# TencentEMapReduce/alluxio

Hardware: AMD Instinct MI355X
Metric: StressWorkerBench cached seq-read GB/s (whole node) at 1/2/4/8 MI355X workers (higher is better)
Workload: dtype uint8; 1 GPU; model=StressWorkerBench cached seq-read, HBM MEM tier, global_batch=256, seq_len=4096, parallelism=workers1, threads_per_worker=256, block_size=67108864, buffer_size=4096, page_size=2097152, verified=True, headline_verified=True, full=False

## Files before the change

### alluxio_amd/csrc/bindings.cpp

```cpp
#include <pybind11/pybind11.h>
#include <pybind11/stl.h>
#include <pybind11/numpy.h>

#include <cmath>
#include <cstring>
#include <vector>

#include "block_store.h"
#include "trace.h"
#include "cpu_codecs.h"
#include "ipc.h"
#include "numa_host.h"
#include "ring_read.h"
#include "ragged_gather.h"
#include "delim_index.h"
#include "field_parse.h"
#include "kernels.h"
#include "seg_ring.h"
#include "frame_rpc.h"
#include "journal_log.h"
#include "meta_codec.h"
#include "fuse_server.h"
#include "http_blob.h"

// ... 820 lines not shown
      .def_property_readonly("passthrough_opens", &FuseServer::passthrough_opens)
      .def("stats", &FuseServer::stats)
      .def_property_readonly("native_opens", &FuseServer::native_opens)
      .def_property_readonly("native_reads", &FuseServer::native_reads)
      .def_property_readonly("fallback_opens", &FuseServer::fallback_opens);
  py::class_<JournalLog>(m, "JournalLog")
      .def(py::init<const std::string&, uint64_t, uint64_t, bool, double>(), py::arg("log_dir"),
           py::arg("next_seq"), py::arg("max_log_bytes"), py::arg("fsync") = true, py::arg("batch_ms") = 5.0)
      .def("append", [](JournalLog& j, py::bytes entry) {
             std::string e = entry;
             return j.append(e);
           })
      .def("request", &JournalLog::request)
      .def("wait_flushed", &JournalLog::wait_flushed, py::arg("counter"), py::arg("timeout_ms") = -1,
           py::call_guard<py::gil_scoped_release>())
      .def("reply_when_flushed", [](JournalLog& j, uint64_t counter, FrameRpcServer& srv, const py::tuple& t) {
             FrameReply r{t[0].cast<uint64_t>(), t[1].cast<int>(), t[2].cast<std::string>(),
                          std::string(t[3].cast<py::bytes>())};
             py::gil_scoped_release rel;
             j.reply_when_flushed(counter, &srv, std::move(r));
           })
      .def("close", &JournalLog::close, py::call_guard<py::gil_scoped_release>())
      .def_property_readonly("next_seq", &JournalLog::next_seq)
      .def_property_readonly("appended", &JournalLog::appended)
      .def_property_readonly("flushed", &JournalLog::flushed)
      .def_property_readonly("error", &JournalLog::error)
      .def_property_readonly("flushes", &JournalLog::flushes)
      .def_property_readonly("segments", &JournalLog::segments)
      .def("stats", &JournalLog::stats);

  py::class_<FrameRpcClient>(m, "FrameRpcClient")
      .def(py::init<const std::string&, int, const std::string&, int>(), py::arg("host"), py::arg("port"),
           py::arg("auth"), py::arg("timeout_ms") = 60000)
      .def("call", [](FrameRpcClient& c, const std::string& path, py::bytes payload, int timeout_ms) {
             std::string p = payload;
             std::tuple<int, std::string, std::string> r;
             {
               py::gil_scoped_release rel;
               r = c.call(path, p, timeout_ms);
             }
             return py::make_tuple(std::get<0>(r), py::str(std::get<1>(r)), py::bytes(std::get<2>(r)));
           }, py::arg("path"), py::arg("payload"), py::arg("timeout_ms") = 0)
      .def("close", &FrameRpcClient::close, G());
  bind_data_path(m);

  m.def("device_count", &hip_device_count);

  m.def("ipc_export", [](uint64_t ptr) {
          IpcExport e = ipc_export(ptr);
          return py::make_tuple(py::bytes(e.handle), e.offset, e.alloc_bytes);
        }, py::arg("ptr"));
  m.def("ipc_open", [](py::bytes handle, int device) {
          std::string h = handle;
          py::gil_scoped_release rel;
          return ipc_open(h, device);
        }, py::arg("handle"), py::arg("device"));
  m.def("ipc_open_bounded", [](py::bytes handle, int device, int timeout_ms) {
          std::string h = handle;
          py::gil_scoped_release rel;
          return ipc_open_bounded(h, device, timeout_ms);
        }, py::arg("handle"), py::arg("device"), py::arg("timeout_ms"));
  py::register_exception<IpcTimeout>(m, "IpcTimeout", PyExc_TimeoutError);
  m.def("ipc_close", [](uint64_t base) { py::gil_scoped_release rel; ipc_close(base); });
  m.def("gpu_numa_node", &gpu_numa_node, py::arg("device"));
  m.def("process_placement", &process_placement);
  m.def("device_arena_alloc", [](uint64_t bytes, int device) {
          py::gil_scoped_release rel;
          return device_arena_alloc(bytes, device);
        }, py::arg("bytes"), py::arg("device"));
  m.def("device_arena_free", [](uint64_t ptr, int device) {
          py::gil_scoped_release rel;
          device_arena_free(ptr, device);
        }, py::arg("ptr"), py::arg("device"));
  m.def("enable_peer_access", &enable_peer_access, py::arg("device"), py::arg("peer"));
  m.def("host_register", [](uint64_t ptr, uint64_t n) {
          if (hip_device_count() == 0) return false;
          HIP_CHECK(hipHostRegister(reinterpret_cast<void*>(ptr), n, hipHostRegisterMapped));
          return true;
        }, py::arg("ptr"), py::arg("nbytes"));
  m.def("host_unregister", [](uint64_t ptr) {
          if (hip_device_count() > 0) (void)hipHostUnregister(reinterpret_cast<void*>(ptr));
        }, py::arg("ptr"));
  m.def("can_access_peer", &can_access_peer, py::arg("device"), py::arg("peer"));
  m.def("crc32c", [](py::buffer data, uint32_t crc) {
          py::buffer_info bi = data.request();
          const size_t n = static_cast<size_t>(bi.size) * bi.itemsize;
          py::gil_scoped_release rel;
          return crc32c_sw(bi.ptr, n, crc);
        }, py::arg("data"), py::arg("crc") = 0);
  m.def("crc32c_ptr", [](uint64_t ptr, uint64_t n, uint32_t crc) {
          py::gil_scoped_release rel;
          return crc32c_sw(reinterpret_cast<const void*>(ptr), n, crc);
        }, py::arg("ptr"), py::arg("n"), py::arg("crc") = 0);
  m.def("crc32c_chunks", [](py::buffer data, uint32_t bpc) {
          py::buffer_info bi = data.request();
          const auto* p = static_cast<const uint8_t*>(bi.ptr);
          const size_t n = static_cast<size_t>(bi.size) * bi.itemsize;
          if (bpc == 0) throw StoreError(kErrInvalidArgument, "bytes_per_checksum must be > 0");
          const size_t nc = (n + bpc - 1) / bpc;
          std::string out(nc * 4, '\0');
          {
            py::gil_scoped_release rel;
            for (size_t i = 0; i < nc; ++i) {
              const size_t off = i * bpc;
              const uint32_t c = crc32c_sw(p + off, std::min<size_t>(bpc, n - off), 0);
              out[4 * i] = char(c >> 24); out[4 * i + 1] = char(c >> 16);
              out[4 * i + 2] = char(c >> 8); out[4 * i + 3] = char(c);
            }
          }
          return py::bytes(out);
        }, py::arg("data"), py::arg("bytes_per_checksum") = 512);
  m.def("crc32c_combine", &crc32c_combine);
  m.def("crc32c_device_pages", &crc32c_device_pages, G(), py::arg("base"), py::arg("pages"), py::arg("length"),
        py::arg("page_bytes"));
  m.def("crc32c_device", &crc32c_device, G(), py::arg("ptr"), py::arg("length"), py::arg("piece") = 0,
        py::arg("stream") = 0);
  m.def("lz4_compress", [](py::bytes data) {
          std::string s = data;
          std::string out(lz4_compress_bound(s.size()), '\0');
          int64_t n;
          {
            py::gil_scoped_release rel;
            n = lz4_compress_block((const uint8_t*)s.data(), s.size(), (uint8_t*)&out[0], out.size());
          }
          if (n < 0) throw StoreError(kErrInvalidArgument, "lz4 compression failed");
          out.resize((size_t)n);
          return py::bytes(out);
        });
  m.def("lz4_decompress", [](py::bytes data, size_t capacity) {
          std::string s = data;
          std::string out(capacity, '\0');
          int64_t n;
          {
            py::gil_scoped_release rel;
            n = lz4_decompress_block((const uint8_t*)s.data(), s.size(), (uint8_t*)&out[0], out.size());
          }
          if (n < 0) throw StoreError(kErrInvalidArgument, "malformed lz4 block (" + std::to_string(n) + ")");
          out.resize((size_t)n);
          return py::bytes(out);
        });
  m.def("lz4_compress_bound", &lz4_compress_bound);
  m.def("trace_push", [](const std::string& name) { roctxRangePushA(name.c_str()); }, py::arg("name"));
  m.def("trace_pop", [] { roctxRangePop(); });
  m.def("trace_mark", [](const std::string& name) { roctxMarkA(name.c_str()); }, py::arg("name"));
  m.def("lz4_device", &lz4_device, G(), py::arg("chunks"), py::arg("compress"), py::arg("stream") = 0);
  m.def("lz4_device_kernel_ms", &lz4_device_kernel_ms, G(), py::arg("chunks"), py::arg("compress"),
        py::arg("reps") = 5);
  m.def("batched_copy", &batched_copy, G(), py::arg("segments"), py::arg("stream") = 0, py::arg("sync") = true);
  m.def("fill_pattern", [](uint64_t ptr, uint64_t bytes, uint64_t seed, uint64_t word_offset, uint64_t stream) {
          py::gil_scoped_release rel;
          HIP_CHECK(launch_fill_pattern(reinterpret_cast<uint8_t*>(ptr), bytes, seed, word_offset,
                                        reinterpret_cast<hipStream_t>(stream)));
        }, py::arg("ptr"), py::arg("bytes"), py::arg("seed"), py::arg("word_offset") = 0, py::arg("stream") = 0);
  m.def("evict_select_device", &evict_select_device);
  m.def("page_alloc_device", &page_alloc_device);
  m.def("set_copy_variant", &set_copy_variant, py::arg("variant"), py::arg("grid_cap") = 0);
  m.def("copy_variant", [] {
    int v = 0;
    unsigned cap = 0;
    copy_variant(&v, &cap);
    return py::make_tuple(v, cap);
  });
  m.def("set_crc_variant", &set_crc_variant, py::arg("variant"));
  m.def("set_lz4_decode_variant", &set_lz4_decode_variant, py::arg("variant"));
  m.def("set_lz4_encode_variant", &set_lz4_encode_variant, py::arg("variant"));
  m.def("set_seq_read_variant", &set_seq_read_variant, py::arg("variant"), py::arg("grid_cap") = 0);
  m.def("seq_read_variant", [] {
    int v = 0;
    unsigned cap = 0;
    seq_read_variant(&v, &cap);
    return py::make_tuple(v, cap);
  });
  m.def("set_ragged_gather_variant", &set_ragged_gather_variant, py::arg("variant"), py::arg("chunk_shift") = 0);
  m.def("ragged_gather_chunk_shift", &ragged_gather_chunk_shift);
  m.def("set_delim_index_variant", &set_delim_index_variant, py::arg("variant"), py::arg("tile_shift") = 0);
  m.def("delim_index_tile_shift", &delim_index_tile_shift);
  m.def("delim_index_variant", &delim_index_variant);
  m.def("set_delim_quote_variant", &set_delim_quote_variant, py::arg("variant"));
  m.def("delim_quote_variant", &delim_quote_variant);
  m.def("set_field_parse_variant", &set_field_parse_variant, py::arg("variant"));
  m.def("field_parse_variant", &field_parse_variant);
  m.def("set_page_gather_chunk_variant", &set_page_gather_chunk_variant, py::arg("variant"));
  m.attr("COPY_CHUNK") = kCopyChunk;
}
```

### alluxio_amd/csrc/kernels.h

```cpp
#pragma once
#include <hip/hip_runtime.h>
#include <cstddef>
#include <cstdint>

#include "field_parse_host.h"

namespace amdx {

struct CopySeg {
  uint64_t src;
  uint64_t dst;
  uint64_t bytes;
  uint64_t chunk0;
};

constexpr uint64_t kCopyChunk = 256 * 1024;

hipError_t launch_batched_copy(const CopySeg* segs, int nseg, uint64_t total_chunks,
                               hipStream_t stream);
void set_copy_variant(int variant, unsigned grid_cap);
void copy_variant(int* variant, unsigned* grid_cap);

struct SeqReadArgs {
  const uint8_t* arena;
  const int64_t* ftab;
  const uint64_t* c_init;
  uint8_t* dst;
  uint64_t stream_stride;
  uint64_t file_len;
  uint64_t buf;
  uint64_t launch_base;
  uint32_t cycle;
  uint32_t streams;
  uint32_t depth;
  uint32_t page_shift;
  uint64_t footprint = 0;
};
constexpr uint32_t kSeqReadMaxStreams = 8192;
hipError_t launch_seq_read(const SeqReadArgs& a, hipStream_t stream);
void set_seq_read_variant(int variant, unsigned grid_cap);
void seq_read_variant(int* variant, unsigned* grid_cap);

struct RaggedRow {
  uint64_t src;
  uint64_t dst_off;
  uint64_t span;
  uint32_t len;
  uint32_t chunk0;
};
struct RaggedRec {
  uint64_t start;
  uint32_t len;
  uint32_t pad;
};
struct RaggedGatherArgs {
  const uint8_t* arena;
  const int64_t* vtab;
  const RaggedRec* recs;
  const int64_t* idx;
  uint8_t* dst;
  uint64_t* out_off;
  uint32_t* out_len;
  RaggedRow* rows;
  uint32_t* chunk_pre;
  uint64_t n_rec;
  uint64_t row_stride;
  uint32_t batch;
  uint32_t page_shift;
  uint32_t align;
  uint32_t max_len;
  uint32_t padded;
  uint32_t pad_value;
  uint32_t total_chunks;
  uint32_t chunk_shift;
};
constexpr uint32_t kRaggedGatherMaxBatch = 65536;
hipError_t launch_ragged_gather(const RaggedGatherArgs& a, hipStream_t stream);
void set_ragged_gather_variant(int variant, unsigned chunk_shift);
uint32_t ragged_gather_chunk_shift();

struct DelimIndexArgs {
  const uint8_t* arena;
  const int64_t* vtab;
  uint32_t* tile_count;
  uint64_t* tile_base;
  uint64_t* out;
  uint64_t out_cap;
  uint64_t vstart;
  uint64_t bytes;
  uint64_t add;
  uint32_t ntiles;
  uint32_t page_shift;
  uint32_t tile_shift;
  uint32_t delim;
  uint32_t quote;
  uint32_t in_quote;
  uint32_t* tile_count_odd;
  uint32_t* tile_parity;
};
uint64_t delim_index_tiles(uint64_t vstart, uint64_t bytes, uint32_t tile_shift);
hipError_t launch_delim_count(const DelimIndexArgs& a, hipStream_t stream);
hipError_t launch_delim_scan(const DelimIndexArgs& a, hipStream_t stream);
hipError_t launch_delim_emit(const DelimIndexArgs& a, uint64_t total, hipStream_t stream);
hipError_t launch_delim_count_quoted(const DelimIndexArgs& a, hipStream_t stream);
hipError_t launch_delim_scan_quoted(const DelimIndexArgs& a, hipStream_t stream);
hipError_t launch_delim_emit_quoted(const DelimIndexArgs& a, uint64_t total, hipStream_t stream);
void set_delim_quote_variant(int variant);
int delim_quote_variant();
void set_delim_index_variant(int variant, unsigned tile_shift);
uint32_t delim_index_tile_shift();
int delim_index_variant();

hipError_t launch_field_parse(const FieldParseArgs& a, hipStream_t stream);
void set_field_parse_variant(int variant);
int field_parse_variant();

hipError_t launch_crc32c_pieces(const uint8_t* base, uint64_t total_bytes, uint64_t piece_bytes,
                                uint32_t* out, uint32_t* scratch, uint64_t scratch_words,
                                hipStream_t stream);
hipError_t launch_crc32c_pages(const uint8_t* base, const int64_t* page_idx, uint64_t total_bytes,
                               uint64_t page_bytes, uint32_t* out, uint32_t* scratch, uint64_t scratch_words,
                               hipStream_t stream);
uint64_t crc32c_pages_scratch_words(uint64_t total_bytes, uint64_t page_bytes);
hipError_t launch_crc32c_gather(const uint64_t* ptrs, const uint32_t* lens, uint64_t n, uint32_t* out,
                                hipStream_t stream);
uint64_t crc32c_gather_max_piece();
void set_crc_variant(int v);
uint64_t crc32c_scratch_words(uint64_t total_bytes, uint64_t piece_bytes);

struct Lz4Chunk {
  uint64_t src;
  uint64_t dst;
  uint32_t src_bytes;
  uint32_t dst_capacity;
};
hipError_t launch_lz4_decompress(const Lz4Chunk* chunks, int n, int32_t* out_sizes,
                                 hipStream_t stream);
void set_lz4_decode_variant(int v);
void set_lz4_encode_variant(int v);
hipError_t launch_lz4_compress(const Lz4Chunk* chunks, int n, int32_t* out_sizes,
                               hipStream_t stream);

struct EvictState {
  float* crf;
  uint64_t* last;
  uint64_t* fbytes;
  int32_t* dir;
  uint32_t n;
  uint64_t now;
  float step;
  float log2_inv_att;
  int policy;
  uint64_t dir_mask;
  int unit;
  int invert;
};
constexpr uint32_t kSlotSetState = 1, kSlotReset = 2, kSlotTouch = 4;
struct SlotUpdate {
  uint32_t slot;
  uint32_t flags;
  int32_t dir;
  float crf;
  uint64_t fbytes;
  uint64_t t;
};
constexpr unsigned kEvSlabRows = 128;
struct EvictCtl {
  unsigned long long hist[256];
  unsigned long long total;
  unsigned long long acc;
  unsigned long long tie_acc;
  unsigned long long freed;
  uint32_t prefix, mask;
  uint32_t all, done;
  uint32_t count, pad;
};
hipError_t launch_slot_update(const EvictState& st, const SlotUpdate* upd, uint32_t n, hipStream_t stream);
hipError_t launch_evict_select_grid(const EvictState& st, uint32_t target_dir, const uint32_t* excl,
                                    uint64_t need, uint32_t* keys, EvictCtl* ctl, uint32_t* out_slots,
                                    hipStream_t stream);
hipError_t launch_page_alloc(uint64_t* bits, uint32_t nwords, uint32_t want, uint32_t* partial,
                             int64_t* pages_out, uint32_t* claimed, hipStream_t stream);
uint32_t page_alloc_partials(uint32_t nwords);

struct ClaimItem {
  uint64_t src;
  uint64_t len;
  uint32_t want;
  uint32_t page_base;
  uint32_t chunk_base;
  uint32_t pad;
};
hipError_t launch_mag_fill(uint64_t* bits, uint32_t nwords, const uint64_t* upd, uint32_t n, hipStream_t stream);
hipError_t launch_mag_drain(uint64_t* bits, uint32_t nwords, uint64_t* out, hipStream_t stream);
// ... 88 lines not shown
```

### alluxio_amd/csrc/kernels.hip

```cpp
#include "kernels.h"

#include <algorithm>
#include <cstring>
#include <mutex>

namespace amdx {

constexpr int kCopyThreads = 256;
typedef unsigned int u32x4 __attribute__((ext_vector_type(4)));

template <int P>
__device__ __forceinline__ u32x4 ld16(const u32x4* p) {
  if constexpr (P == 1) return __builtin_nontemporal_load(p);
  else return *p;
}
template <int P>
__device__ __forceinline__ void st16(u32x4* p, u32x4 v) {
  if constexpr (P == 1) __builtin_nontemporal_store(v, p);
  else *p = v;
}

__device__ __forceinline__ void copy_bytes(const uint8_t* __restrict__ s, uint8_t* __restrict__ d,
                                           uint64_t n, int tid) {
  for (uint64_t i = tid; i < n; i += kCopyThreads) d[i] = s[i];
}

template <int UNROLL, int LP, int SP>
__device__ __forceinline__ void copy_range(uint64_t src, uint64_t dst, uint64_t n, int tid) {
  if (((src | dst) & 15) == 0) {
    const u32x4* __restrict__ s = reinterpret_cast<const u32x4*>(src);
    u32x4* __restrict__ d = reinterpret_cast<u32x4*>(dst);
    const uint64_t n16 = n >> 4;
    uint64_t i = tid;
    constexpr uint64_t kStep = (uint64_t)kCopyThreads * UNROLL;
    for (; i + (UNROLL - 1) * kCopyThreads < n16; i += kStep) {
      u32x4 v[UNROLL];
#pragma unroll
      for (int u = 0; u < UNROLL; ++u) v[u] = ld16<LP>(s + i + (uint64_t)u * kCopyThreads);
#pragma unroll
      for (int u = 0; u < UNROLL; ++u) st16<SP>(d + i + (uint64_t)u * kCopyThreads, v[u]);
    }
    for (; i < n16; i += kCopyThreads) st16<SP>(d + i, ld16<LP>(s + i));
    const uint64_t done = n16 << 4;
    if (done < n) copy_bytes(reinterpret_cast<const uint8_t*>(src) + done,
                             reinterpret_cast<uint8_t*>(dst) + done, n - done, tid);
  } else if (((src | dst) & 3) == 0) {
    const uint32_t* __restrict__ s = reinterpret_cast<const uint32_t*>(src);
    uint32_t* __restrict__ d = reinterpret_cast<uint32_t*>(dst);
    const uint64_t n4 = n >> 2;
    for (uint64_t i = tid; i < n4; i += kCopyThreads) d[i] = s[i];
    const uint64_t done = n4 << 2;
    if (done < n) copy_bytes(reinterpret_cast<const uint8_t*>(src) + done,
                             reinterpret_cast<uint8_t*>(dst) + done, n - done, tid);
  } else {
    copy_bytes(reinterpret_cast<const uint8_t*>(src), reinterpret_cast<uint8_t*>(dst), n, tid);
  }
}

template <int UNROLL, int LP, int SP>
__global__ __launch_bounds__(kCopyThreads) void batched_copy_kernel(
    const CopySeg* __restrict__ segs, int nseg, uint64_t total_chunks) {
  const int tid = threadIdx.x;
  for (uint64_t c = blockIdx.x; c < total_chunks; c += gridDim.x) {
    int lo = 0, hi = nseg - 1;
    while (lo < hi) {
      const int mid = (lo + hi + 1) >> 1;
      if (segs[mid].chunk0 <= c) lo = mid; else hi = mid - 1;
    }
    lo = __builtin_amdgcn_readfirstlane(lo);
    const uint64_t src = segs[lo].src, dst = segs[lo].dst, bytes = segs[lo].bytes;
    const uint64_t off = (c - segs[lo].chunk0) * kCopyChunk;
    const uint64_t n = bytes - off < kCopyChunk ? bytes - off : kCopyChunk;
    copy_range<UNROLL, LP, SP>(src + off, dst + off, n, tid);
  }
}

static int g_copy_variant = 8;
static unsigned g_copy_grid_cap = 4096;

void set_copy_variant(int variant, unsigned grid_cap) {
  g_copy_variant = variant;
  if (grid_cap) g_copy_grid_cap = grid_cap;
}
void copy_variant(int* variant, unsigned* grid_cap) {
  *variant = g_copy_variant;
  *grid_cap = g_copy_grid_cap;
}

hipError_t launch_batched_copy(const CopySeg* segs, int nseg, uint64_t total_chunks,
                               hipStream_t stream) {
  if (nseg <= 0 || total_chunks == 0) return hipSuccess;
  const dim3 grid((unsigned)std::min<uint64_t>(total_chunks, g_copy_grid_cap));
  const dim3 block(kCopyThreads);
#define AMDX_COPY(U, L, S) hipLaunchKernelGGL((batched_copy_kernel<U, L, S>), grid, block, 0, stream, segs, nseg, total_chunks)
  switch (g_copy_variant) {
    case 1: AMDX_COPY(8, 0, 1); break;
    case 2: AMDX_COPY(8, 1, 0); break;
    case 3: AMDX_COPY(8, 1, 1); break;
    case 4: AMDX_COPY(4, 0, 0); break;
    case 5: AMDX_COPY(4, 0, 1); break;
    case 8: AMDX_COPY(16, 0, 0); break;
    case 9: AMDX_COPY(16, 0, 1); break;
    default: AMDX_COPY(8, 0, 0); break;
  }
#undef AMDX_COPY
  return hipGetLastError();
}

constexpr int kSeqThreads = 256;

template <bool POW2, int UNROLL, int SP, int LP>
__global__ __launch_bounds__(kSeqThreads) void seq_read_kernel(SeqReadArgs a, uint32_t vpr_shift,
                                                               uint32_t depth_shift) {
  extern __shared__ uint32_t c0[];
  for (uint32_t s = threadIdx.x; s < a.streams; s += kSeqThreads)
    c0[s] = (uint32_t)((a.c_init[s] + a.launch_base) % a.cycle);
  __syncthreads();
  const uint64_t vpr = a.buf >> 4;
  const uint64_t nvec = (uint64_t)a.streams * a.depth * vpr;
  const uint64_t pmask = (1ull << a.page_shift) - 1;
  const uint64_t gstride = (uint64_t)gridDim.x * kSeqThreads;
  for (uint64_t base = (uint64_t)blockIdx.x * kSeqThreads + threadIdx.x; base < nvec;
       base += gstride * UNROLL) {
    u32x4 v[UNROLL];
    uint8_t* d[UNROLL];
    uint32_t nb[UNROLL];
#pragma unroll
    for (int u = 0; u < UNROLL; ++u) {
      const uint64_t i = base + (uint64_t)u * gstride;
      nb[u] = 0;
      d[u] = nullptr;
      if (i >= nvec) continue;
      uint64_t r, vi;
      uint32_t s, k;
      if constexpr (POW2) {
        r = i >> vpr_shift;
        vi = i & (vpr - 1);
        s = (uint32_t)(r >> depth_shift);
        k = (uint32_t)(r & (a.depth - 1));
      } else {
        r = i / vpr;
        vi = i - r * vpr;
        s = (uint32_t)(r / a.depth);
        k = (uint32_t)(r - (uint64_t)s * a.depth);
      }
      uint32_t c = c0[s] + k;
      if (c >= a.cycle) c = (uint32_t)(((uint64_t)c0[s] + k) % a.cycle);
      if (c == a.cycle - 1) continue;
      const uint64_t off = (uint64_t)c * a.buf + vi * 16;
      const uint64_t rend = ((uint64_t)c + 1) * a.buf;
      const uint64_t end = rend < a.file_len ? rend : a.file_len;
      if (off >= end) continue;
      const uint64_t page = (uint64_t)a.ftab[off >> a.page_shift];
      const uint8_t* src = a.arena + (page << a.page_shift) + (off & pmask);
      d[u] = a.dst + (uint64_t)s * a.stream_stride + (uint64_t)k * a.buf + vi * 16;
      if (end - off >= 16) {
        nb[u] = 16;
        v[u] = ld16<LP>(reinterpret_cast<const u32x4*>(src));
      } else {
        nb[u] = (uint32_t)(end - off);
        for (uint32_t b = 0; b < nb[u]; ++b) {
          const uint64_t o = off + b;
          d[u][b] = a.arena[((uint64_t)a.ftab[o >> a.page_shift] << a.page_shift) + (o & pmask)];
        }
      }
    }
#pragma unroll
    for (int u = 0; u < UNROLL; ++u)
      if (nb[u] == 16) st16<SP>(reinterpret_cast<u32x4*>(d[u]), v[u]);
  }
}

static int g_seq_variant = -1;
static unsigned g_seq_grid_cap = 8192;

void set_seq_read_variant(int variant, unsigned grid_cap) {
  g_seq_variant = variant;
  if (grid_cap) g_seq_grid_cap = grid_cap;
}
void seq_read_variant(int* variant, unsigned* grid_cap) {
  *variant = g_seq_variant;
  *grid_cap = g_seq_grid_cap;
}

static inline bool is_pow2(uint64_t x) { return x && !(x & (x - 1)); }
static inline uint32_t log2u(uint64_t x) {
  uint32_t s = 0;
  while ((1ull << s) < x) ++s;
  return s;
}

hipError_t launch_seq_read(const SeqReadArgs& a, hipStream_t stream) {
  if (a.streams == 0 || a.depth == 0 || a.buf == 0 || a.file_len == 0) return hipSuccess;
  if (a.streams > kSeqReadMaxStreams || (a.buf & 15) || (a.stream_stride & 15) ||
      ((uint64_t)a.dst & 15) || ((uint64_t)a.arena & 15))
    return hipErrorInvalidValue;
  const uint64_t vpr = a.buf >> 4;
  const uint64_t nvec = (uint64_t)a.streams * a.depth * vpr;
  const uint64_t fp = a.footprint ? a.footprint : a.file_len;
  const int var = g_seq_variant >= 0 ? g_seq_variant : (fp >= (128ull << 20) ? 4 : 0);
  const int unroll = (var & 2) ? 16 : 8;
  uint64_t blocks = (nvec + (uint64_t)kSeqThreads * unroll - 1) / ((uint64_t)kSeqThreads * unroll);
  if (blocks > g_seq_grid_cap) blocks = g_seq_grid_cap;
  if (blocks < 1) blocks = 1;
  const bool p2 = is_pow2(vpr) && is_pow2(a.depth);
  const uint32_t vs = log2u(vpr), ds = log2u(a.depth);
  const size_t lds = a.streams * sizeof(uint32_t);
  const dim3 g((unsigned)blocks), b(kSeqThreads);
#define AMDX_SEQ(P2, U, SP, LP) \
  hipLaunchKernelGGL((seq_read_kernel<P2, U, SP, LP>), g, b, lds, stream, a, vs, ds)
  const int sp = var & 1, lp = (var >> 2) & 1;
  if (p2) {
    if (unroll == 16) {
      if (lp) { if (sp) AMDX_SEQ(true, 16, 1, 1); else AMDX_SEQ(true, 16, 0, 1); }
      else { if (sp) AMDX_SEQ(true, 16, 1, 0); else AMDX_SEQ(true, 16, 0, 0); }
    } else {
      if (lp) { if (sp) AMDX_SEQ(true, 8, 1, 1); else AMDX_SEQ(true, 8, 0, 1); }
      else { if (sp) AMDX_SEQ(true, 8, 1, 0); else AMDX_SEQ(true, 8, 0, 0); }
    }
  } else {
    if (lp) { if (sp) AMDX_SEQ(false, 8, 1, 1); else AMDX_SEQ(false, 8, 0, 1); }
    else { if (sp) AMDX_SEQ(false, 8, 1, 0); else AMDX_SEQ(false, 8, 0, 0); }
  }
#undef AMDX_SEQ
  return hipGetLastError();
}

constexpr uint32_t kCrcPoly = 0x82F63B78u;
constexpr uint64_t kCrcSeg = 64 * 1024;
constexpr int kCrcThreads = 256;
constexpr uint64_t kCrcLane = kCrcSeg / kCrcThreads;

__constant__ uint32_t c_crc_tab[8][256];
__constant__ uint32_t c_x2n[64];
__constant__ uint32_t c_crc16[16][256];
__constant__ uint32_t c_shift4k[4][256];
__constant__ uint32_t c_lane_shift[256];
constexpr int kCrc4Threads = 1024;
__constant__ uint32_t c_crc11[12][2048];
__constant__ uint32_t c_shift16k[4][256];
__constant__ uint32_t c_lane_shift1k[kCrc4Threads];
constexpr int kCrc5Threads = 1024;
constexpr uint64_t kCrc5Chunk = 64;
__constant__ uint32_t c_shift5[4][256];
__constant__ uint32_t c_lane_shift5[kCrc5Threads];

static void host_crc_tables(uint32_t tab[8][256], uint32_t x2n[64]) {
  for (uint32_t i = 0; i < 256; ++i) {
    uint32_t c = i;
    for (int k = 0; k < 8; ++k) c = (c & 1) ? (c >> 1) ^ kCrcPoly : c >> 1;
    tab[0][i] = c;
  }
  for (int t = 1; t < 8; ++t)
    for (uint32_t i = 0; i < 256; ++i) tab[t][i] = (tab[t - 1][i] >> 8) ^ tab[0][tab[t - 1][i] & 0xFF];
  auto mult = [](uint32_t a, uint32_t b) {
    uint32_t m = 1u << 31, p = 0;
    for (;;) {
      if (a & m) { p ^= b; if ((a & (m - 1)) == 0) break; }
      m >>= 1;
      b = (b & 1) ? (b >> 1) ^ kCrcPoly : b >> 1;
    }
    return p;
  };
  uint32_t p = 1u << 30;
  x2n[0] = p;
  for (int k = 1; k < 64; ++k) { p = mult(p, p); x2n[k] = p; }
}

static uint32_t host_gf2_mult(uint32_t a, uint32_t b) {
  uint32_t p = 0;
  for (uint32_t m = 1u << 31; m; m >>= 1) {
    if (a & m) p ^= b;
    b = (b & 1) ? (b >> 1) ^ kCrcPoly : b >> 1;
  }
  return p;
}

static void host_crc16_tables(const uint32_t tab8[8][256], const uint32_t x2n[64], uint32_t t16[16][256],
                              uint32_t sh[4][256]) {
  for (uint32_t i = 0; i < 256; ++i) t16[0][i] = tab8[0][i];
  for (int t = 1; t < 16; ++t)
    for (uint32_t i = 0; i < 256; ++i) t16[t][i] = (t16[t - 1][i] >> 8) ^ t16[0][t16[t - 1][i] & 0xFF];
  const uint32_t k = x2n[15];
  for (int b = 0; b < 4; ++b)
    for (uint32_t i = 0; i < 256; ++i) sh[b][i] = host_gf2_mult(k, i << (8 * b));
}

static std::once_flag g_crc_once;
static hipError_t g_crc_init_err = hipSuccess;

static hipError_t ensure_crc_tables() {
  std::call_once(g_crc_once, [] {
    static uint32_t tab[8][256];
    static uint32_t x2n[64];
    host_crc_tables(tab, x2n);
    static uint32_t t16[16][256];
    static uint32_t sh[4][256];
    host_crc16_tables(tab, x2n, t16, sh);
    g_crc_init_err = hipMemcpyToSymbol(HIP_SYMBOL(c_crc_tab), tab, sizeof(tab));
    if (g_crc_init_err == hipSuccess)
      g_crc_init_err = hipMemcpyToSymbol(HIP_SYMBOL(c_x2n), x2n, sizeof(x2n));
    if (g_crc_init_err == hipSuccess)
      g_crc_init_err = hipMemcpyToSymbol(HIP_SYMBOL(c_crc16), t16, sizeof(t16));
    if (g_crc_init_err == hipSuccess)
      g_crc_init_err = hipMemcpyToSymbol(HIP_SYMBOL(c_shift4k), sh, sizeof(sh));
    static uint32_t t11[12][2048];
    uint32_t e[128];
    for (int k = 0; k < 128; ++k) e[k] = t16[15 - k / 8][1u << (k % 8)];
    for (int c = 0; c < 12; ++c)
      for (uint32_t v = 0; v < 2048; ++v) {
        uint32_t x = 0;
        for (int b = 0; b < 11; ++b)
          if (((v >> b) & 1) && 11 * c + b < 128) x ^= e[11 * c + b];
        t11[c][v] = x;
      }
    static uint32_t sh16k[4][256];
    for (int b = 0; b < 4; ++b)
      for (uint32_t i = 0; i < 256; ++i) sh16k[b][i] = host_gf2_mult(x2n[17], i << (8 * b));
    static uint32_t lane1k[kCrc4Threads];
    lane1k[0] = 1u << 31;
    for (int k = 1; k < kCrc4Threads; ++k) lane1k[k] = host_gf2_mult(lane1k[k - 1], x2n[7]);
    if (g_crc_init_err == hipSuccess)
      g_crc_init_err = hipMemcpyToSymbol(HIP_SYMBOL(c_crc11), t11, sizeof(t11));
    if (g_crc_init_err == hipSuccess)
      g_crc_init_err = hipMemcpyToSymbol(HIP_SYMBOL(c_shift16k), sh16k, sizeof(sh16k));
    if (g_crc_init_err == hipSuccess)
      g_crc_init_err = hipMemcpyToSymbol(HIP_SYMBOL(c_lane_shift1k), lane1k, sizeof(lane1k));
    {
      const uint64_t nbits = 8ull * (kCrc5Threads - 1) * kCrc5Chunk;
      uint32_t k5 = 1u << 31;
      for (int b = 0; b < 64; ++b)
        if ((nbits >> b) & 1) k5 = host_gf2_mult(x2n[b], k5);
      static uint32_t sh5[4][256];
      for (int b = 0; b < 4; ++b)
        for (uint32_t i = 0; i < 256; ++i) sh5[b][i] = host_gf2_mult(k5, i << (8 * b));
      static uint32_t lane5[kCrc5Threads];
      lane5[0] = 1u << 31;
      for (int d = 1; d < kCrc5Threads; ++d) lane5[d] = host_gf2_mult(lane5[d - 1], x2n[9]);
      if (g_crc_init_err == hipSuccess)
        g_crc_init_err = hipMemcpyToSymbol(HIP_SYMBOL(c_shift5), sh5, sizeof(sh5));
      if (g_crc_init_err == hipSuccess)
        g_crc_init_err = hipMemcpyToSymbol(HIP_SYMBOL(c_lane_shift5), lane5, sizeof(lane5));
    }
    static uint32_t lane_shift[256];
    lane_shift[0] = 1u << 31;
    for (int k = 1; k < 256; ++k) lane_shift[k] = host_gf2_mult(lane_shift[k - 1], x2n[7]);
    if (g_crc_init_err == hipSuccess)
      g_crc_init_err = hipMemcpyToSymbol(HIP_SYMBOL(c_lane_shift), lane_shift, sizeof(lane_shift));
  });
  return g_crc_init_err;
}

__device__ __forceinline__ uint32_t gf2_mult(uint32_t a, uint32_t b) {
  uint32_t m = 1u << 31, p = 0;
  for (int i = 0; i < 32; ++i) {
    if (a & m) p ^= b;
    m >>= 1;
    b = (b & 1) ? (b >> 1) ^ kCrcPoly : b >> 1;
  }
  return p;
}

__device__ __forceinline__ uint32_t xpow8n(uint64_t nbytes) {
  uint64_t n = nbytes << 3;
  uint32_t p = 1u << 31;
  int k = 0;
  while (n) {
    if (n & 1) p = gf2_mult(c_x2n[k & 63], p);
    n >>= 1;
    ++k;
  }
  return p;
}

__global__ __launch_bounds__(kCrcThreads) void crc32c_segments_kernel(
    const uint8_t* __restrict__ base, uint64_t total_bytes, uint64_t piece_bytes,
    uint64_t segs_per_piece, uint64_t nsegs, uint32_t* __restrict__ seg_crc) {
// ... 2453 lines not shown
```

### alluxio_amd/csrc/ring_read.cpp

```cpp
#include "ring_read.h"

#include <algorithm>
#include <cstring>
#include <string>

#include "kernels.h"

namespace amdx {

RingReadSession::RingReadSession(BlockStore* store, int64_t session, const std::vector<int64_t>& block_ids,
                                 const std::vector<uint64_t>& block_lens, uint64_t dst_base,
                                 uint64_t stream_stride, uint64_t buf_bytes, uint32_t depth, uint32_t streams,
                                 int dst_kind, const std::vector<uint64_t>& start_offsets)
    : store_(store), session_(session), blocks_(block_ids), pins_(store), buf_(buf_bytes), stride_(stream_stride),
      dst_(dst_base), depth_(depth), streams_(streams), kind_(dst_kind) {
  if (block_ids.size() != block_lens.size() || block_ids.empty())
    throw StoreError(kErrInvalidArgument, "ring read: bad block list");
  for (uint64_t l : block_lens) file_len_ += l;
  check_shape();
  view_.append_file(store_, pins_, session_, blocks_, block_lens, "ring read");
  on_device_ = store_->has_device();
  finish_init(start_offsets);
}

RingReadSession::RingReadSession(uint64_t arena_base, const std::vector<int64_t>& file_pages, uint64_t page_size,
                                 uint64_t file_len, int device, uint64_t dst_base, uint64_t stream_stride,
                                 uint64_t buf_bytes, uint32_t depth, uint32_t streams, int dst_kind,
                                 const std::vector<uint64_t>& start_offsets)
    : store_(nullptr), session_(0), pins_(nullptr), file_len_(file_len), buf_(buf_bytes), stride_(stream_stride),
      dst_(dst_base), depth_(depth), streams_(streams), kind_(dst_kind), on_device_(device >= 0), device_(device) {
  check_shape();
  view_ = PagedView::raw(arena_base, file_pages, page_size, device, "ring read");
  if (view_.vtab.size() < (file_len_ + page_size - 1) / page_size)
    throw StoreError(kErrInvalidArgument, "ring read: page table shorter than the file");
  finish_init(start_offsets);
}

void RingReadSession::check_shape() {
  if (buf_ == 0 || depth_ == 0 || streams_ == 0 || streams_ > kSeqReadMaxStreams)
    throw StoreError(kErrInvalidArgument, "ring read: bad buffer/depth/stream count");
  if (stride_ < (uint64_t)depth_ * buf_) throw StoreError(kErrInvalidArgument, "ring read: stride too small");
  if (file_len_ == 0) throw StoreError(kErrInvalidArgument, "ring read: empty file");
  const uint64_t calls = (file_len_ + buf_ - 1) / buf_;
  if (calls + 1 >= (1ull << 32)) throw StoreError(kErrInvalidArgument, "ring read: too many calls per pass");
  cycle_ = (uint32_t)(calls + 1);
}

void RingReadSession::set_device() const {
  if (store_) store_->use_device();
  else if (device_ >= 0) AMDX_HIP(hipSetDevice(device_));
}

void RingReadSession::finish_init(const std::vector<uint64_t>& start_offsets) {
  c_init_.assign(streams_, 0);
  for (uint32_t s = 0; s < streams_ && s < start_offsets.size(); ++s) {
    if (start_offsets[s] % buf_) throw StoreError(kErrInvalidArgument, "ring read: start offsets must be buffer aligned");
    c_init_[s] = std::min<uint64_t>(start_offsets[s] / buf_, cycle_ - 1);
  }
  std::vector<uint64_t> starts(c_init_);
  std::sort(starts.begin(), starts.end());
  const uint64_t distinct = (uint64_t)(std::unique(starts.begin(), starts.end()) - starts.begin());
  footprint_ = std::min<uint64_t>(file_len_, distinct * depth_ * buf_);
  if (on_device_) {
    if (buf_ & 15 || stride_ & 15 || dst_ & 15)
      throw StoreError(kErrInvalidArgument, "ring read: buffer size, stride and ring base must be 16-byte aligned");
    set_device();
    d_ftab_.alloc(view_.vtab.size() * sizeof(int64_t));
    d_cinit_.alloc(c_init_.size() * sizeof(uint64_t));
    AMDX_HIP(hipMemcpy(d_ftab_.p, view_.vtab.data(), view_.vtab.size() * sizeof(int64_t), hipMemcpyHostToDevice));
    AMDX_HIP(hipMemcpy(d_cinit_.p, c_init_.data(), c_init_.size() * sizeof(uint64_t), hipMemcpyHostToDevice));
  }
}

RingReadSession::~RingReadSession() {
  try {
    close();
  } catch (...) {
  }
}

void RingReadSession::close() {
  if (closed_) return;
  closed_ = true;
  d_ftab_.reset();
  d_cinit_.reset();
  pins_.release();
}

uint64_t RingReadSession::bytes_before(uint64_t g) const {
  const uint64_t passes = g / cycle_, rem = g % cycle_;
  return passes * file_len_ + std::min<uint64_t>(rem * buf_, file_len_);
}

uint64_t RingReadSession::step(uint64_t stream, uint64_t* eofs) {
  if (closed_) throw StoreError(kErrInvalidState, "ring read session closed");
  const uint64_t base = calls_per_stream_;
  if (on_device_) {
    set_device();
    SeqReadArgs a;
    a.arena = view_.base();
    a.ftab = d_ftab_.as<int64_t>();
    a.c_init = d_cinit_.as<uint64_t>();
    a.dst = reinterpret_cast<uint8_t*>(dst_);
    a.stream_stride = stride_;
    a.file_len = file_len_;
    a.buf = buf_;
    a.launch_base = base;
    a.cycle = cycle_;
    a.streams = streams_;
    a.depth = depth_;
    a.page_shift = view_.page_shift;
    a.footprint = footprint_;
    hipStream_t st = reinterpret_cast<hipStream_t>(stream);
    AMDX_HIP(launch_seq_read(a, st));
    if (kind_ == (int)MemKind::kHost) AMDX_HIP(hipStreamSynchronize(st));
  } else {
    for (uint32_t s = 0; s < streams_; ++s)
      for (uint32_t k = 0; k < depth_; ++k) {
        auto [off, len] = std::pair<uint64_t, uint64_t>(0, 0);
        const uint64_t c = (c_init_[s] + base + k) % cycle_;
        if (c == cycle_ - 1) continue;
        off = c * buf_;
        len = std::min(buf_, file_len_ - off);
        uint8_t* d = reinterpret_cast<uint8_t*>(dst_ + s * stride_ + (uint64_t)k * buf_);
        for_each_page_run(view_.base(), view_.vtab.data(), view_.page_shift, off, len,
                          [d](const uint8_t* p, uint64_t n, uint64_t done) { std::memcpy(d + done, p, n); });
      }
  }
  uint64_t bytes = 0, eof = 0;
  for (uint32_t s = 0; s < streams_; ++s) {
    const uint64_t g0 = c_init_[s] + base, g1 = g0 + depth_;
    bytes += bytes_before(g1) - bytes_before(g0);
    eof += g1 / cycle_ - g0 / cycle_;
  }
  calls_per_stream_ += depth_;
  total_ += bytes;
  reopens_ += eof;
  if (store_) store_->access_blocks(blocks_);
  if (eofs) *eofs = eof;
  return bytes;
}

uint64_t RingReadSession::position(uint32_t s) const {
  const uint64_t c = (c_init_.at(s) + calls_per_stream_) % cycle_;
  return std::min<uint64_t>(c * buf_, file_len_);
}

std::pair<uint64_t, uint64_t> RingReadSession::last_call(uint32_t s, uint32_t k) const {
  if (calls_per_stream_ < depth_) return {0, 0};
  const uint64_t c = (c_init_.at(s) + calls_per_stream_ - depth_ + k) % cycle_;
  if (c == cycle_ - 1) return {file_len_, 0};
  const uint64_t off = c * buf_;
  return {off, std::min(buf_, file_len_ - off)};
}

}
```

### alluxio_amd/csrc/ring_read.h

```cpp
#pragma once
#include <cstdint>
#include <vector>

#include "paged_view.h"

namespace amdx {

class RingReadSession {
 public:
  RingReadSession(BlockStore* store, int64_t session, const std::vector<int64_t>& block_ids,
                  const std::vector<uint64_t>& block_lens, uint64_t dst_base, uint64_t stream_stride,
                  uint64_t buf_bytes, uint32_t depth, uint32_t streams, int dst_kind,
                  const std::vector<uint64_t>& start_offsets);
  RingReadSession(uint64_t arena_base, const std::vector<int64_t>& file_pages, uint64_t page_size,
                  uint64_t file_len, int device, uint64_t dst_base, uint64_t stream_stride, uint64_t buf_bytes,
                  uint32_t depth, uint32_t streams, int dst_kind, const std::vector<uint64_t>& start_offsets);
  ~RingReadSession();
  uint64_t step(uint64_t stream, uint64_t* eofs);
  void close();
  uint64_t total_bytes() const { return total_; }
  uint64_t reopens() const { return reopens_; }
  uint64_t calls() const { return calls_per_stream_; }
  uint64_t position(uint32_t s) const;
  std::pair<uint64_t, uint64_t> last_call(uint32_t s, uint32_t k) const;
  uint64_t file_len() const { return file_len_; }

 private:
  uint64_t bytes_before(uint64_t g) const;
  void check_shape();
  void finish_init(const std::vector<uint64_t>& start_offsets);
  void set_device() const;
  BlockStore* store_;
  int64_t session_;
  std::vector<int64_t> blocks_;
  BlockPins pins_;
  uint64_t file_len_ = 0, buf_, stride_, dst_;
  uint32_t depth_, streams_, cycle_;
  int kind_;
  bool on_device_ = false;
  int device_ = -1;
  PagedView view_;
  std::vector<uint64_t> c_init_;
  uint64_t footprint_ = 0;
  DevBuf d_ftab_, d_cinit_;
  uint64_t calls_per_stream_ = 0, total_ = 0, reopens_ = 0;
  bool closed_ = false;
};

}
```

Before: 5878 GB/s.

## Add wave-per-chunk fast seq-read kernel with persistent grid and modular call base

Adds a new seq-read kernel in which each wavefront copies U contiguous 1 KiB chunks. When the run stays inside one page and one call, a single page-table lookup serves all U loads; otherwise it falls back to a per-chunk path. The grid is capped at the occupancy-derived resident workgroup count, and the host keeps a modular base so the kernel avoids 64-bit modulo per element. It also computes the byte accounting in a closed form for lockstep streams and adds a store-fill probe kernel, at the cost of many extra template instantiations and more complex index arithmetic.

Result: faster. 6510 GB/s, median of 6 (+10.8%).

```diff
diff --git a/alluxio_amd/csrc/bindings.cpp b/alluxio_amd/csrc/bindings.cpp
--- a/alluxio_amd/csrc/bindings.cpp
+++ b/alluxio_amd/csrc/bindings.cpp
@@ -996,6 +996,15 @@
           HIP_CHECK(launch_fill_pattern(reinterpret_cast<uint8_t*>(ptr), bytes, seed, word_offset,
                                         reinterpret_cast<hipStream_t>(stream)));
         }, py::arg("ptr"), py::arg("bytes"), py::arg("seed"), py::arg("word_offset") = 0, py::arg("stream") = 0);
+  m.def("store_fill", [](uint64_t ptr, uint64_t bytes, uint32_t word, bool nontemporal, unsigned grid,
+                         uint64_t stream) {
+          py::gil_scoped_release rel;
+          unsigned used = 0;
+          HIP_CHECK(launch_store_fill(reinterpret_cast<uint8_t*>(ptr), bytes, word, nontemporal, grid, &used,
+                                      reinterpret_cast<hipStream_t>(stream)));
+          return used;
+        }, py::arg("ptr"), py::arg("bytes"), py::arg("word") = 0, py::arg("nontemporal") = false,
+        py::arg("grid") = 0, py::arg("stream") = 0);
   m.def("evict_select_device", &evict_select_device);
   m.def("page_alloc_device", &page_alloc_device);
   m.def("set_copy_variant", &set_copy_variant, py::arg("variant"), py::arg("grid_cap") = 0);
@@ -1015,6 +1024,10 @@
     seq_read_variant(&v, &cap);
     return py::make_tuple(v, cap);
   });
+  m.def("seq_read_last_launch", [] {
+    const SeqReadLaunch l = seq_read_last_launch();
+    return py::make_tuple(l.fast ? "fast" : "general", l.unroll, l.grid);
+  });
   m.def("set_ragged_gather_variant", &set_ragged_gather_variant, py::arg("variant"), py::arg("chunk_shift") = 0);
   m.def("ragged_gather_chunk_shift", &ragged_gather_chunk_shift);
   m.def("set_delim_index_variant", &set_delim_index_variant, py::arg("variant"), py::arg("tile_shift") = 0);
diff --git a/alluxio_amd/csrc/kernels.h b/alluxio_amd/csrc/kernels.h
--- a/alluxio_amd/csrc/kernels.h
+++ b/alluxio_amd/csrc/kernels.h
@@ -35,11 +35,20 @@
   uint32_t depth;
   uint32_t page_shift;
   uint64_t footprint = 0;
+  uint64_t base_mod = ~0ull;
 };
 constexpr uint32_t kSeqReadMaxStreams = 8192;
 hipError_t launch_seq_read(const SeqReadArgs& a, hipStream_t stream);
 void set_seq_read_variant(int variant, unsigned grid_cap);
 void seq_read_variant(int* variant, unsigned* grid_cap);
+struct SeqReadLaunch {
+  int fast;
+  int unroll;
+  unsigned grid;
+};
+SeqReadLaunch seq_read_last_launch();
+hipError_t launch_store_fill(uint8_t* dst, uint64_t bytes, uint32_t word, bool nontemporal, unsigned grid,
+                             unsigned* grid_used, hipStream_t stream);
 
 struct RaggedRow {
   uint64_t src;
diff --git a/alluxio_amd/csrc/kernels.hip b/alluxio_amd/csrc/kernels.hip
--- a/alluxio_amd/csrc/kernels.hip
+++ b/alluxio_amd/csrc/kernels.hip
@@ -108,6 +108,8 @@
 }
 
 constexpr int kSeqThreads = 256;
+constexpr uint32_t kSeqChunkShift = 10;
+constexpr uint32_t kSeqChunk = 1u << kSeqChunkShift;
 
 template <bool POW2, int UNROLL, int SP, int LP>
 __global__ __launch_bounds__(kSeqThreads) void seq_read_kernel(SeqReadArgs a, uint32_t vpr_shift,
@@ -171,6 +173,117 @@
   }
 }
 
+template <bool POW2>
+__device__ __forceinline__ void seq_split(const SeqReadArgs& a, uint64_t q, uint64_t cpr, uint32_t cpr_shift,
+                                          uint32_t depth_shift, uint32_t* s, uint32_t* k, uint64_t* ci) {
+  if constexpr (POW2) {
+    const uint64_t rd = q >> cpr_shift;
+    *ci = q & (cpr - 1);
+    *s = (uint32_t)(rd >> depth_shift);
+    *k = (uint32_t)(rd & (a.depth - 1));
+  } else {
+    const uint64_t rd = q / cpr;
+    *ci = q - rd * cpr;
+    *s = (uint32_t)(rd / a.depth);
+    *k = (uint32_t)(rd - (uint64_t)*s * a.depth);
+  }
+}
+
+template <bool MULTI>
+__device__ __forceinline__ uint64_t seq_call_index(const SeqReadArgs& a, uint64_t c0, uint32_t k) {
+  if constexpr (MULTI) k %= a.cycle;
+  uint64_t c = c0 + a.base_mod;
+  c = c >= a.cycle ? c - a.cycle : c;
+  c += k;
+  return c >= a.cycle ? c - a.cycle : c;
+}
+
+template <bool POW2, int U, int SP, int LP, bool MULTI>
+__device__ __forceinline__ void seq_fast_loop(const SeqReadArgs& a, const uint8_t* __restrict__ arena,
+                                              const int64_t* __restrict__ ftab,
+                                              const uint64_t* __restrict__ c_init, uint8_t* __restrict__ dst,
+                                              uint32_t cpr_shift, uint32_t depth_shift) {
+  constexpr uint32_t kWaves = kSeqThreads / 64;
+  constexpr uint64_t kTrip = (uint64_t)U * kSeqChunk;
+  constexpr int kGen = 4;
+  const uint32_t lane16 = (threadIdx.x & 63u) * 16u;
+  const uint32_t wave = (uint32_t)__builtin_amdgcn_readfirstlane((int)(threadIdx.x >> 6));
+  const uint64_t cpr = a.buf >> kSeqChunkShift;
+  const uint64_t per_stream = (uint64_t)a.depth * cpr;
+  const uint64_t nchunks = (uint64_t)a.streams * per_stream;
+  const uint64_t ngroups = (nchunks + U - 1) / U;
+  const uint64_t nwaves = (uint64_t)gridDim.x * kWaves;
+  const uint64_t pmask = (1ull << a.page_shift) - 1;
+  for (uint64_t g = (uint64_t)blockIdx.x * kWaves + wave; g < ngroups; g += nwaves) {
+    uint32_t s0, k0;
+    uint64_t ci0;
+    seq_split<POW2>(a, g * U, cpr, cpr_shift, depth_shift, &s0, &k0, &ci0);
+    const uint64_t w0 = (uint64_t)k0 * cpr + ci0;
+    const uint64_t off0 = seq_call_index<MULTI>(a, c_init[s0], k0) * a.buf + (ci0 << kSeqChunkShift);
+    u32x4 v[U];
+    if (w0 + U <= per_stream && off0 + kTrip <= a.file_len && (off0 & pmask) + kTrip <= pmask + 1) {
+      const uint64_t page = (uint64_t)ftab[off0 >> a.page_shift];
+      const u32x4* sp = reinterpret_cast<const u32x4*>(arena + (page << a.page_shift) + (off0 & pmask) + lane16);
+      u32x4* dp = reinterpret_cast<u32x4*>(dst + (uint64_t)s0 * a.stream_stride + (w0 << kSeqChunkShift) + lane16);
+#pragma unroll
+      for (int u = 0; u < U; ++u) v[u] = ld16<LP>(sp + u * (kSeqChunk / 16));
+#pragma unroll
+      for (int u = 0; u < U; ++u) st16<SP>(dp + u * (kSeqChunk / 16), v[u]);
+      continue;
+    }
+#pragma unroll 1
+    for (int h = 0; h < U; h += kGen) {
+      uint64_t dof[kGen], c0[kGen], sof[kGen];
+      uint32_t k[kGen], n[kGen];
+      int64_t page[kGen];
+#pragma unroll
+      for (int u = 0; u < kGen; ++u) {
+        const uint64_t q = g * U + h + u;
+        n[u] = q < nchunks ? kSeqChunk : 0;
+        uint32_t s;
+        uint64_t ci;
+        seq_split<POW2>(a, q < nchunks ? q : 0, cpr, cpr_shift, depth_shift, &s, &k[u], &ci);
+        sof[u] = ci << kSeqChunkShift;
+        dof[u] = (uint64_t)s * a.stream_stride + (uint64_t)k[u] * a.buf + sof[u];
+        c0[u] = c_init[s];
+      }
+#pragma unroll
+      for (int u = 0; u < kGen; ++u) {
+        const uint64_t c = seq_call_index<MULTI>(a, c0[u], k[u]);
+        const uint64_t off = c * a.buf + sof[u];
+        const bool data = c != a.cycle - 1 && off < a.file_len;
+        const uint64_t left = data ? a.file_len - off : 0;
+        n[u] = left < n[u] ? (uint32_t)left : n[u];
+        sof[u] = data ? off : 0;
+        page[u] = ftab[sof[u] >> a.page_shift];
+      }
+#pragma unroll
+      for (int u = 0; u < kGen; ++u) {
+        const uint8_t* src = arena + ((uint64_t)page[u] << a.page_shift) + (sof[u] & pmask);
+        sof[u] = reinterpret_cast<uint64_t>(src);
+        if (lane16 + 16 <= n[u]) v[u] = ld16<LP>(reinterpret_cast<const u32x4*>(src + lane16));
+      }
+#pragma unroll
+      for (int u = 0; u < kGen; ++u) {
+        if (lane16 + 16 <= n[u]) {
+          st16<SP>(reinterpret_cast<u32x4*>(dst + dof[u] + lane16), v[u]);
+        } else if (lane16 < n[u]) {
+          const uint8_t* src = reinterpret_cast<const uint8_t*>(sof[u]);
+          for (uint32_t b = lane16; b < n[u]; ++b) dst[dof[u] + b] = src[b];
+        }
+      }
+    }
+  }
+}
+
+template <bool POW2, int U, int SP, int LP>
+__global__ __launch_bounds__(kSeqThreads) void seq_read_fast_kernel(
+    SeqReadArgs a, const uint8_t* __restrict__ arena, const int64_t* __restrict__ ftab,
+    const uint64_t* __restrict__ c_init, uint8_t* __restrict__ dst, uint32_t cpr_shift, uint32_t depth_shift) {
+  if (a.depth > a.cycle) seq_fast_loop<POW2, U, SP, LP, true>(a, arena, ftab, c_init, dst, cpr_shift, depth_shift);
+  else seq_fast_loop<POW2, U, SP, LP, false>(a, arena, ftab, c_init, dst, cpr_shift, depth_shift);
+}
+
 static int g_seq_variant = -1;
 static unsigned g_seq_grid_cap = 8192;
 
@@ -182,12 +295,61 @@
   *variant = g_seq_variant;
   *grid_cap = g_seq_grid_cap;
 }
+
+static SeqReadLaunch g_seq_last;
+
+SeqReadLaunch seq_read_last_launch() { return g_seq_last; }
 
 static inline bool is_pow2(uint64_t x) { return x && !(x & (x - 1)); }
 static inline uint32_t log2u(uint64_t x) {
   uint32_t s = 0;
   while ((1ull << s) < x) ++s;
   return s;
+}
+
+constexpr int kMaxDev = 64;
+template <typename K>
+static hipError_t resident_workgroups(K kernel, unsigned (&cached)[kMaxDev], unsigned* out) {
+  static std::mutex mu;
+  int dev = 0;
+  hipError_t e = hipGetDevice(&dev);
+  if (e != hipSuccess) return e;
+  if (dev < 0 || dev >= kMaxDev) return hipErrorInvalidDevice;
+  std::lock_guard<std::mutex> lk(mu);
+  if (!cached[dev]) {
+    int cus = 0, per_cu = 0;
+    if ((e = hipDeviceGetAttribute(&cus, hipDeviceAttributeMultiprocessorCount, dev)) != hipSuccess) return e;
+    if ((e = hipOccupancyMaxActiveBlocksPerMultiprocessor(&per_cu, kernel, kSeqThreads, 0)) != hipSuccess) return e;
+    if (cus < 1 || per_cu < 1) return hipErrorInvalidValue;
+    cached[dev] = (unsigned)cus * (unsigned)per_cu;
+  }
+  *out = cached[dev];
+  return hipSuccess;
+}
+
+template <bool P2, int U, int SP, int LP>
+static hipError_t seq_fast_resident(unsigned* out) {
+  static unsigned cached[kMaxDev] = {};
+  return resident_workgroups(seq_read_fast_kernel<P2, U, SP, LP>, cached, out);
+}
+
+template <bool P2, int U, int SP, int LP>
+static hipError_t launch_seq_fast(const SeqReadArgs& a, hipStream_t stream) {
+  unsigned resident = 0;
+  const hipError_t e = seq_fast_resident<P2, U, SP, LP>(&resident);
+  if (e != hipSuccess) return e;
+  const uint64_t cpr = a.buf >> kSeqChunkShift;
+  const uint64_t nchunks = (uint64_t)a.streams * a.depth * cpr;
+  const uint64_t ngroups = (nchunks + U - 1) / U;
+  constexpr uint64_t kWaves = kSeqThreads / 64;
+  uint64_t blocks = (ngroups + kWaves - 1) / kWaves;
+  if (blocks > resident) blocks = resident;
+  if (blocks > g_seq_grid_cap) blocks = g_seq_grid_cap;
+  if (blocks < 1) blocks = 1;
+  hipLaunchKernelGGL((seq_read_fast_kernel<P2, U, SP, LP>), dim3((unsigned)blocks), dim3(kSeqThreads), 0, stream,
+                     a, a.arena, a.ftab, a.c_init, a.dst, log2u(cpr), log2u(a.depth));
+  g_seq_last = SeqReadLaunch{1, U, (unsigned)blocks};
+  return hipGetLastError();
 }
 
 hipError_t launch_seq_read(const SeqReadArgs& a, hipStream_t stream) {
@@ -200,6 +362,20 @@
   const uint64_t fp = a.footprint ? a.footprint : a.file_len;
   const int var = g_seq_variant >= 0 ? g_seq_variant : (fp >= (128ull << 20) ? 4 : 0);
   const int unroll = (var & 2) ? 16 : 8;
+  if ((a.buf & (kSeqChunk - 1)) == 0 && a.page_shift >= kSeqChunkShift && a.base_mod < a.cycle) {
+    const bool p2 = is_pow2(a.buf >> kSeqChunkShift) && is_pow2(a.depth);
+    const int sel = (p2 ? 8 : 0) | (unroll == 16 ? 4 : 0) | ((var & 1) ? 2 : 0) | ((var & 4) ? 1 : 0);
+    switch (sel) {
+#define AMDX_FAST(N, P2, U, SP, LP) case N: return launch_seq_fast<P2, U, SP, LP>(a, stream)
+      AMDX_FAST(0, false, 8, 0, 0); AMDX_FAST(1, false, 8, 0, 1); AMDX_FAST(2, false, 8, 1, 0);
+      AMDX_FAST(3, false, 8, 1, 1); AMDX_FAST(4, false, 16, 0, 0); AMDX_FAST(5, false, 16, 0, 1);
+      AMDX_FAST(6, false, 16, 1, 0); AMDX_FAST(7, false, 16, 1, 1); AMDX_FAST(8, true, 8, 0, 0);
+      AMDX_FAST(9, true, 8, 0, 1); AMDX_FAST(10, true, 8, 1, 0); AMDX_FAST(11, true, 8, 1, 1);
+      AMDX_FAST(12, true, 16, 0, 0); AMDX_FAST(13, true, 16, 0, 1); AMDX_FAST(14, true, 16, 1, 0);
+      default: AMDX_FAST(15, true, 16, 1, 1);
+#undef AMDX_FAST
+    }
+  }
   uint64_t blocks = (nvec + (uint64_t)kSeqThreads * unroll - 1) / ((uint64_t)kSeqThreads * unroll);
   if (blocks > g_seq_grid_cap) blocks = g_seq_grid_cap;
   if (blocks < 1) blocks = 1;
@@ -223,6 +399,51 @@
     else { if (sp) AMDX_SEQ(false, 8, 1, 0); else AMDX_SEQ(false, 8, 0, 0); }
   }
 #undef AMDX_SEQ
+  g_seq_last = SeqReadLaunch{0, p2 ? unroll : 8, (unsigned)blocks};
+  return hipGetLastError();
+}
+
+template <int SP>
+__global__ __launch_bounds__(kSeqThreads) void store_fill_kernel(u32x4* __restrict__ dst, uint64_t nvec,
+                                                                 uint32_t word) {
+  constexpr uint32_t kWaves = kSeqThreads / 64;
+  constexpr uint64_t kTripVec = 8 * (kSeqChunk / 16);
+  const u32x4 v = {word, word, word, word};
+  const uint32_t lane = threadIdx.x & 63u;
+  const uint32_t wave = (uint32_t)__builtin_amdgcn_readfirstlane((int)(threadIdx.x >> 6));
+  const uint64_t trips = nvec / kTripVec;
+  const uint64_t nwaves = (uint64_t)gridDim.x * kWaves;
+  for (uint64_t g = (uint64_t)blockIdx.x * kWaves + wave; g < trips; g += nwaves) {
+    u32x4* p = dst + g * kTripVec + lane;
+#pragma unroll
+    for (int u = 0; u < 8; ++u) st16<SP>(p + u * (kSeqChunk / 16), v);
+  }
+  for (uint64_t i = trips * kTripVec + (uint64_t)blockIdx.x * kSeqThreads + threadIdx.x; i < nvec;
+       i += (uint64_t)gridDim.x * kSeqThreads)
+    st16<SP>(dst + i, v);
+}
+
+hipError_t launch_store_fill(uint8_t* dst, uint64_t bytes, uint32_t word, bool nontemporal, unsigned grid,
+                             unsigned* grid_used, hipStream_t stream) {
+  if (((uint64_t)dst & 15) || (bytes & 15)) return hipErrorInvalidValue;
+  if (grid_used) *grid_used = 0;
+  if (bytes == 0) return hipSuccess;
+  static unsigned cached[2][kMaxDev] = {};
+  unsigned resident = 0;
+  const hipError_t e = nontemporal ? resident_workgroups(store_fill_kernel<1>, cached[1], &resident)
+                                   : resident_workgroups(store_fill_kernel<0>, cached[0], &resident);
+  if (e != hipSuccess) return e;
+  const uint64_t nvec = bytes >> 4;
+  uint64_t blocks = grid ? grid : resident;
+  const uint64_t need = (nvec + kSeqThreads - 1) / kSeqThreads;
+  if (blocks > need) blocks = need;
+  if (nontemporal)
+    hipLaunchKernelGGL(store_fill_kernel<1>, dim3((unsigned)blocks), dim3(kSeqThreads), 0, stream,
+                       reinterpret_cast<u32x4*>(dst), nvec, word);
+  else
+    hipLaunchKernelGGL(store_fill_kernel<0>, dim3((unsigned)blocks), dim3(kSeqThreads), 0, stream,
+                       reinterpret_cast<u32x4*>(dst), nvec, word);
+  if (grid_used) *grid_used = (unsigned)blocks;
   return hipGetLastError();
 }
 
diff --git a/alluxio_amd/csrc/ring_read.cpp b/alluxio_amd/csrc/ring_read.cpp
--- a/alluxio_amd/csrc/ring_read.cpp
+++ b/alluxio_amd/csrc/ring_read.cpp
@@ -44,6 +44,8 @@
   const uint64_t calls = (file_len_ + buf_ - 1) / buf_;
   if (calls + 1 >= (1ull << 32)) throw StoreError(kErrInvalidArgument, "ring read: too many calls per pass");
   cycle_ = (uint32_t)(calls + 1);
+  full_passes_ = depth_ / cycle_;
+  rem_calls_ = depth_ % cycle_;
 }
 
 void RingReadSession::set_device() const {
@@ -61,6 +63,7 @@
   std::sort(starts.begin(), starts.end());
   const uint64_t distinct = (uint64_t)(std::unique(starts.begin(), starts.end()) - starts.begin());
   footprint_ = std::min<uint64_t>(file_len_, distinct * depth_ * buf_);
+  lockstep_ = distinct == 1;
   if (on_device_) {
     if (buf_ & 15 || stride_ & 15 || dst_ & 15)
       throw StoreError(kErrInvalidArgument, "ring read: buffer size, stride and ring base must be 16-byte aligned");
@@ -87,9 +90,14 @@
   pins_.release();
 }
 
-uint64_t RingReadSession::bytes_before(uint64_t g) const {
-  const uint64_t passes = g / cycle_, rem = g % cycle_;
-  return passes * file_len_ + std::min<uint64_t>(rem * buf_, file_len_);
+uint64_t RingReadSession::step_bytes(uint64_t c0, uint64_t* eofs) const {
+  auto before = [this](uint64_t x) {
+    return x < cycle_ ? std::min<uint64_t>(x * buf_, file_len_)
+                      : file_len_ + std::min<uint64_t>((x - cycle_) * buf_, file_len_);
+  };
+  const uint64_t c1 = c0 + rem_calls_;
+  *eofs = (uint64_t)full_passes_ + (c1 >= cycle_ ? 1 : 0);
+  return (uint64_t)full_passes_ * file_len_ + before(c1) - before(c0);
 }
 
 uint64_t RingReadSession::step(uint64_t stream, uint64_t* eofs) {
@@ -106,6 +114,7 @@
     a.file_len = file_len_;
     a.buf = buf_;
     a.launch_base = base;
+    a.base_mod = base_mod_;
     a.cycle = cycle_;
     a.streams = streams_;
     a.depth = depth_;
@@ -118,7 +127,7 @@
     for (uint32_t s = 0; s < streams_; ++s)
       for (uint32_t k = 0; k < depth_; ++k) {
         auto [off, len] = std::pair<uint64_t, uint64_t>(0, 0);
-        const uint64_t c = (c_init_[s] + base + k) % cycle_;
+        const uint64_t c = (c_init_[s] + base_mod_ + k) % cycle_;
         if (c == cycle_ - 1) continue;
         off = c * buf_;
         len = std::min(buf_, file_len_ - off);
@@ -127,13 +136,24 @@
                           [d](const uint8_t* p, uint64_t n, uint64_t done) { std::memcpy(d + done, p, n); });
       }
   }
+  auto first_call = [this](uint32_t s) {
+    const uint64_t c = c_init_[s] + base_mod_;
+    return c >= cycle_ ? c - cycle_ : c;
+  };
   uint64_t bytes = 0, eof = 0;
-  for (uint32_t s = 0; s < streams_; ++s) {
-    const uint64_t g0 = c_init_[s] + base, g1 = g0 + depth_;
-    bytes += bytes_before(g1) - bytes_before(g0);
-    eof += g1 / cycle_ - g0 / cycle_;
+  if (lockstep_) {
+    bytes = step_bytes(first_call(0), &eof) * streams_;
+    eof *= streams_;
+  } else {
+    for (uint32_t s = 0; s < streams_; ++s) {
+      uint64_t e = 0;
+      bytes += step_bytes(first_call(s), &e);
+      eof += e;
+    }
   }
   calls_per_stream_ += depth_;
+  base_mod_ += rem_calls_;
+  if (base_mod_ >= cycle_) base_mod_ -= cycle_;
   total_ += bytes;
   reopens_ += eof;
   if (store_) store_->access_blocks(blocks_);
diff --git a/alluxio_amd/csrc/ring_read.h b/alluxio_amd/csrc/ring_read.h
--- a/alluxio_amd/csrc/ring_read.h
+++ b/alluxio_amd/csrc/ring_read.h
@@ -26,7 +26,7 @@
   uint64_t file_len() const { return file_len_; }
 
  private:
-  uint64_t bytes_before(uint64_t g) const;
+  uint64_t step_bytes(uint64_t c0, uint64_t* eofs) const;
   void check_shape();
   void finish_init(const std::vector<uint64_t>& start_offsets);
   void set_device() const;
@@ -42,6 +42,9 @@
   PagedView view_;
   std::vector<uint64_t> c_init_;
   uint64_t footprint_ = 0;
+  bool lockstep_ = false;
+  uint32_t full_passes_ = 0, rem_calls_ = 0;
+  uint64_t base_mod_ = 0;
   DevBuf d_ftab_, d_cinit_;
   uint64_t calls_per_stream_ = 0, total_ = 0, reopens_ = 0;
   bool closed_ = false;
```
